# Ameek94/BOBE

Measured on AMD Instinct MI355X. Metric: GP fit+acquisition cycles/sec at N=4096 d=8, 65536 cands; Cholesky GF/s, higher is better.
Workload: dtype f64

## Files before the change

### bobe_amd/csrc/chol_kernels.hpp

```cpp
#pragma once
#include "kernels_common.hpp"

namespace bobe {

constexpr int PLD = 130;
constexpr int POTF2_DLD = 17;

template <bool LOWER = false, int NWAVES = 4>
__device__ __forceinline__ void block_load(double* S, const double* __restrict__ G, int64_t ld) {
  const int lane = threadIdx.x & 63, wave = threadIdx.x >> 6;
  constexpr int NI = TILE / NWAVES;
  v2d v[NI];
#pragma unroll
  for (int i = 0; i < NI; ++i) {
    const int r = NWAVES * i + wave;
    const int c = LOWER ? ((2 * lane <= r) ? 2 * lane : (r & ~1)) : 2 * lane;
    v[i] = *reinterpret_cast<const v2d*>(G + (int64_t)r * ld + c);
  }
#pragma unroll
  for (int i = 0; i < NI; ++i) *reinterpret_cast<v2d*>(S + (NWAVES * i + wave) * PLD + 2 * lane) = v[i];
}
__device__ __forceinline__ void block_store_lower(const double* S, double* __restrict__ G, int64_t ld) {
  const int lane = threadIdx.x & 63, wave = threadIdx.x >> 6;
#pragma unroll 8
// ... 598 lines not shown
}

__global__ __launch_bounds__(256) void k_copy_diag(double* __restrict__ A, int64_t lda, int64_t bsA,
                                                   const double* __restrict__ diag, int64_t bsD, int first) {
  const int blk = first + blockIdx.x;
  const double* src = diag + blockIdx.y * bsD + (int64_t)blk * TILE * TILE;
  double* dst = A + blockIdx.y * bsA + ((int64_t)blk * TILE) * lda + (int64_t)blk * TILE;
  const int lane = threadIdx.x & 63, wave = threadIdx.x >> 6;
#pragma unroll 8
  for (int i = 0; i < 32; ++i) {
    const int r = 4 * i + wave;
    *reinterpret_cast<v2d*>(dst + (int64_t)r * lda + 2 * lane) = *reinterpret_cast<const v2d*>(src + r * TILE + 2 * lane);
  }
}

template <int T, int BK>
__global__ __launch_bounds__(256) void k_syrk_trail(double* __restrict__ A, int64_t lda, int k0, int k1, int first,
                                                    int colmode, int n, int64_t bsA = 0, int per = 0,
                                                    const int* __restrict__ colk0 = nullptr, int far_col = 0, int ncol = 0) {
  extern __shared__ double smem[];
  A += blockIdx.y * bsA;
  int a, b;
  if (colmode == 0) {
    if (per > 0) {
      const int t = xcd_share(blockIdx.x, per);
      if (t >= n * (n + 1) / 2) return;
      tri_grouped(t, n, a, b);
    } else {
      tri_decode(blockIdx.x, a, b);
    }
  } else {
    const int S = colmode == 1 ? TILE / T : ncol;
// ... 2 lines not shown
    for (int c = 0; c < S - 1; ++c)
      if (b == c && idx >= n - c) {
        idx -= n - c;
        b = c + 1;
      }
    a = b + idx;
  }
  if (colk0) {
    const int col = first + (b * T) / TILE;
    if (col >= far_col) k0 = colk0[col];
    if (k0 >= k1) return;
  }
  const int64_t base = (int64_t)first * TILE;
  v4d acc[T / 32][T / 32];
  load_tile<T, T>(acc, A, lda, base + (int64_t)a * T, base + (int64_t)b * T);
  gemm_tile<KC, KC, T, T, BK, true>(acc, A, lda, base + (int64_t)a * T, A, lda, base + (int64_t)b * T,
                                    (int64_t)k0 * TILE, (int64_t)k1 * TILE, smem);
  store_tile<T, T>(acc, A, lda, base + (int64_t)a * T, base + (int64_t)b * T, 1.0, 0.0);
}


template <int T>
__device__ __forceinline__ bool tri_find(const TriProb* __restrict__ probs, int nprob, int bid, TriProb& p, int& e0,
                                         int& e1) {
  constexpr int S = (TILE / T) * (TILE / T);
  for (int q = 0; q < nprob; ++q) {
    const TriProb c = probs[q];
    const int nt = (c.hi - c.mid) * (c.mid - c.lo) * S;
    const int nw = (T == 128) ? nt : nt / 2;
    const int o = (T == 128) ? c.off : c.off * S / 2;
    if (bid >= o && bid < o + nw) {
      p = c;
      e0 = bid - o;
      e1 = (T == 128) ? -1 : nt - 1 - e0;
      return true;
    }
  }
  return false;
}

template <int T>
__global__ __launch_bounds__(256, 2) void k_trtri_T(const double* __restrict__ L, int64_t ldl,
                                                    const double* __restrict__ Linv, int64_t ldi,
                                                    double* __restrict__ Tmp, int64_t ldt,
                                                    const TriProb* __restrict__ probs, int nprob, int64_t bsA = 0,
                                                    int64_t bsL = 0, int64_t bsT = 0, int per = 0) {
  extern __shared__ double smem[];
  L += blockIdx.y * bsA;
  Linv += blockIdx.y * bsL;
  Tmp += blockIdx.y * bsT;
  TriProb p;
  int e[2];
  if (!tri_find<T>(probs, nprob, xcd_share(blockIdx.x, per), p, e[0], e[1])) return;
  const int rows = (p.hi - p.mid) * (TILE / T), w = (p.mid - p.lo) * (TILE / T);
  for (int u = 0; u < 2; ++u) {
    if (e[u] < 0) continue;
    int ti, tj;
    if (per > 0) {
      rect_grouped(e[u], w, rows, tj, ti);
    } else {
      tj = e[u] / rows, ti = e[u] % rows;
    }
    const int64_t m0 = (int64_t)p.mid * TILE + (int64_t)ti * T, n0 = (int64_t)p.lo * TILE + (int64_t)tj * T;
    v4d acc[T / 32][T / 32];
    acc_zero(acc);
    gemm_tile<KC, RC, T, T, TileCfg<T>::bk>(acc, L, ldl, m0, Linv, ldi, n0, n0, (int64_t)p.mid * TILE, smem);
    store_tile<T, T>(acc, Tmp, ldt, m0, n0, 1.0, 0.0);
  }
}

template <int T>
__global__ __launch_bounds__(256, 2) void k_trtri_R(double* __restrict__ Linv, int64_t ldi,
                                                    const double* __restrict__ Tmp, int64_t ldt,
                                                    const TriProb* __restrict__ probs, int nprob, int64_t bsL = 0,
                                                    int64_t bsT = 0, int per = 0) {
  extern __shared__ double smem[];
  Linv += blockIdx.y * bsL;
  Tmp += blockIdx.y * bsT;
  TriProb p;
  int e[2];
  if (!tri_find<T>(probs, nprob, xcd_share(blockIdx.x, per), p, e[0], e[1])) return;
  const int rows = (p.hi - p.mid) * (TILE / T), w = (p.mid - p.lo) * (TILE / T);
  for (int u = 0; u < 2; ++u) {
    if (e[u] < 0) continue;
    int ti, tj;
    if (per > 0) {
      rect_grouped(e[u], rows, w, ti, tj);
      ti = rows - 1 - ti;
    } else {
      ti = rows - 1 - e[u] / w, tj = e[u] % w;
    }
    const int64_t m0 = (int64_t)p.mid * TILE + (int64_t)ti * T, n0 = (int64_t)p.lo * TILE + (int64_t)tj * T;
    v4d acc[T / 32][T / 32];
    acc_zero(acc);
    gemm_tile<KC, RC, T, T, TileCfg<T>::bk>(acc, Linv, ldi, m0, Tmp, ldt, n0, (int64_t)p.mid * TILE, m0 + T, smem);
    store_tile<T, T>(acc, Linv, ldi, m0, n0, -1.0, 0.0);
  }
}

__global__ __launch_bounds__(256, 2) void k_lauum_tiles32(const double* __restrict__ Linv, int64_t ldi, int64_t np,
                                                          double* __restrict__ Kinv, int64_t ldk, int64_t bsL, int64_t bsK,
                                                          int nbatch) {
  extern __shared__ double smem[];
  const int tile = (int)(blockIdx.x / nbatch), slot = (int)(blockIdx.x % nbatch);
  Linv += slot * bsL;
  Kinv += slot * bsK;
  int ti, tj;
  tri_decode(tile >> 2, ti, tj);
  const int r32 = 2 * ti + ((tile >> 1) & 1), c32 = 2 * tj + (tile & 1);
  v4d acc[1][1];
  acc_zero(acc);
  gemm_tile<RC, RC, 32, 32, BK32>(acc, Linv, ldi, (int64_t)r32 * 32, Linv, ldi, (int64_t)c32 * 32,
                                  (int64_t)(r32 > c32 ? r32 : c32) * 32, np, smem);
  store_tile<32, 32>(acc, Kinv, ldk, (int64_t)r32 * 32, (int64_t)c32 * 32, 1.0, 0.0);
}

template <int KERN, int DCAP, int T>
__global__ __launch_bounds__(256, 2) void k_lauum_grad(const double* __restrict__ Linv, int64_t ldi, int64_t np,
                                                       int64_t n, const double* __restrict__ alpha,
                                                       const double* __restrict__ XsT, int64_t ldx, Hyper h,
                                                       double* __restrict__ partial, double* __restrict__ Kinv,
                                                       int64_t ldk, const Hyper* __restrict__ hp = nullptr,
                                                       int64_t bsL = 0, int64_t bsV = 0, int64_t bsX = 0,
                                                       int64_t bsP = 0, int nbatch = 1, int from_kinv = 0, int64_t bsK = 0) {
  extern __shared__ double smem[];
  const int tile = (int)(blockIdx.x / nbatch), slot = (int)(blockIdx.x % nbatch);
  if (hp) h = hp[slot];
  Linv += slot * bsL;
  alpha += slot * bsV;
  XsT += slot * bsX;
  partial += slot * bsP;
  int ti, tj;
  tri_decode(tile, ti, tj);
  v4d acc[T / 32][T / 32];
  if (from_kinv) {
    load_tile<T, T>(acc, Kinv + slot * bsK, ldk, (int64_t)ti * T, (int64_t)tj * T);
  } else {
    acc_zero(acc);
    gemm_tile<RC, RC, T, T, TileCfg<T>::bk>(acc, Linv, ldi, (int64_t)ti * T, Linv, ldi, (int64_t)tj * T, (int64_t)ti * T, np,
                                            smem);
    if (Kinv) store_tile<T, T>(acc, Kinv, ldk, (int64_t)ti * T, (int64_t)tj * T, 1.0, 0.0);
  }
  double* xa = smem;
  double* xb = smem + MAX_D * T;
  double* aa = smem + 2 * MAX_D * T;
  double* ab = aa + T;
  double* red = ab + T;
  const int t = threadIdx.x;
  for (int e = t; e < h.d * T; e += 256) {
    const int j = e / T, c = e % T;
    xa[j * T + c] = XsT[j * ldx + (int64_t)ti * T + c];
    xb[j * T + c] = XsT[j * ldx + (int64_t)tj * T + c];
  }
  if (t < T) {
    aa[t] = alpha[(int64_t)ti * T + t];
// ... 51 lines not shown
```

### bobe_amd/csrc/gemm_f64.hpp

```cpp
#pragma once
#include <hip/hip_runtime.h>
#include <stdint.h>
#include <type_traits>

namespace bobe {

typedef double v4d __attribute__((ext_vector_type(4)));
typedef double v2d __attribute__((ext_vector_type(2)));

constexpr int TILE = 128;
constexpr int TK = 16;
constexpr int GEMM_THREADS = 256;

enum Layout { KC = 0, RC = 1 };

template <int L, int R, int BK>
struct Img {
  static constexpr int stride = (L == KC) ? (BK + 2) : (R + 16);
  static constexpr int doubles = (L == KC) ? R * (BK + 2) : BK * (R + 16);
};
constexpr int imax(int a, int b) { return a > b ? a : b; }
template <int TM, int TN, int BK>
constexpr int gemm_smem_doubles() {
  return 2 * (imax(Img<KC, TM, BK>::doubles, Img<RC, TM, BK>::doubles) +
// ... 307 lines not shown
    BOBE_STAMP_STEP();
    buf ^= 1;
    frags(fa[0], fb[0], smem + buf * (IA + IB), 0);
    __builtin_amdgcn_sched_barrier(0);
    mfmas(BK / 4 - 1);
    __builtin_amdgcn_sched_barrier(0);
    BOBE_STAMP(0);
  };
  const int64_t kd = TRIL ? (kend - TM > kbeg ? kend - TM : kbeg) : kend;
  for (int64_t k0 = kbeg; k0 < kd; k0 += BK) kstep(k0, std::false_type(), 0);
  if (TRIL)
    for (int64_t k0 = kd; k0 < kend; k0 += BK) kstep(k0, std::true_type(), (int)(k0 - (kend - TM)));
  BOBE_STAMPS_END(tid);
}

template <int TM = 128>
__device__ __forceinline__ int acc_row(int i, int r, int tid = threadIdx.x) {
  const int t = tid;
  return ((t >> 6) >> 1) * (TM / 2) + 16 * i + ((t & 63) >> 4) + 4 * r;
}
template <int TN = 128>
__device__ __forceinline__ int acc_col(int j, int tid = threadIdx.x) {
  const int t = tid;
  return ((t >> 6) & 1) * (TN / 2) + 16 * j + (t & 15);
}

template <int TM = 128, int TN = 128>
__device__ __forceinline__ void store_tile(const v4d (&acc)[TM / 32][TN / 32], double* __restrict__ C, int64_t ldc,
                                           int64_t m0, int64_t n0, double alpha, double beta, int tid = threadIdx.x) {
#pragma unroll
// ... 63 lines not shown
```

### bobe_amd/csrc/gp_factor.hip

```cpp
#include "gp_handle.hpp"

#include <chrono>

#include "chol_kernels.hpp"

using namespace bobe;

namespace bobe {

constexpr int SYRK32_BK = 128, SYRK64_BK = 16;
constexpr int SYRK32_SMEM = gemm_smem_doubles_exact<KC, KC, 32, 32, SYRK32_BK>() * 8 / 2;
constexpr int SYRK64_SMEM = gemm_smem_doubles_exact<KC, KC, 64, 64, SYRK64_BK>() * 8;

void configure_factor_kernels() {
  static bool done[64] = {false};
  int dev = 0;
  HIPCHK(hipGetDevice(&dev));
  if (dev < 0 || dev >= 64 || done[dev]) return;
  allow_big_lds(k_potf2<true>, POTF2_SMEM_BYTES);
  allow_big_lds(k_potf2<false>, POTF2_SMEM_BYTES);
  allow_big_lds(k_trti_diag, POTF2_SMEM_BYTES);
  allow_big_lds(k_trsm_panel, TRSM_SMEM_BYTES);
  allow_big_lds((k_chol_panel<false, 3>), POTF2_SMEM_BYTES);
  allow_big_lds((k_chol_panel<false, 4>), POTF2_SMEM_BYTES);
  allow_big_lds((k_chol_panel<true, 3>), POTF2_SMEM_BYTES);
  allow_big_lds((k_chol_panel<true, 4>), POTF2_SMEM_BYTES);
  allow_big_lds(k_trtri_T<128>, GEMM_SMEM_BYTES);
  allow_big_lds(k_trtri_R<128>, GEMM_SMEM_BYTES);
  allow_big_lds(k_syrk_trail<64, SYRK64_BK>, SYRK64_SMEM);
  allow_big_lds(k_syrk_trail<32, SYRK32_BK>, SYRK32_SMEM);
  allow_big_lds(k_trtri_T<64>, GEMM64_SMEM_BYTES);
  allow_big_lds(k_trtri_R<64>, GEMM64_SMEM_BYTES);
  allow_big_lds(k_trtri_T<32>, GEMM32_SMEM_BYTES);
  allow_big_lds(k_trtri_R<32>, GEMM32_SMEM_BYTES);
  allow_big_lds(k_lauum_tiles32, GEMM32_SMEM_BYTES);
  allow_big_lds(k_lauum_grad<0, 8, 64>, GEMM64_SMEM_BYTES);
  allow_big_lds(k_lauum_grad<0, 16, 64>, GEMM64_SMEM_BYTES);
  allow_big_lds(k_lauum_grad<0, 32, 64>, GEMM64_SMEM_BYTES);
  allow_big_lds(k_lauum_grad<1, 8, 64>, GEMM64_SMEM_BYTES);
  allow_big_lds(k_lauum_grad<1, 16, 64>, GEMM64_SMEM_BYTES);
  allow_big_lds(k_lauum_grad<1, 32, 64>, GEMM64_SMEM_BYTES);
  allow_big_lds(k_lauum_grad<0, 8, 128>, GEMM_SMEM_BYTES);
  allow_big_lds(k_lauum_grad<0, 16, 128>, GEMM_SMEM_BYTES);
  allow_big_lds(k_lauum_grad<0, 32, 128>, GEMM_SMEM_BYTES);
  allow_big_lds(k_lauum_grad<1, 8, 128>, GEMM_SMEM_BYTES);
  allow_big_lds(k_lauum_grad<1, 16, 128>, GEMM_SMEM_BYTES);
  allow_big_lds(k_lauum_grad<1, 32, 128>, GEMM_SMEM_BYTES);
  done[dev] = true;
}

const Tuning& tuning() {
  static Tuning t = [] {
    Tuning v{512, 600, 300, 1, BOBE_MAX_MLL_SLOTS, 2048, 1, 1, false, false, true, true};
    auto geti = [](const char* name, int& dst) {
      const char* e = std::getenv(name);
      if (e) dst = std::atoi(e);
      return e != nullptr;
    };
    geti("BOBE_SYRK32_BELOW", v.syrk32_below);
    geti("BOBE_TRTRI64", v.trtri64_below);
    geti("BOBE_PAIR_MIN", v.pair_min);
    geti("BOBE_LOCKSTEP_MIN_N", v.lockstep_min_n);
    v.mll_slots_set = geti("BOBE_MLL_SLOTS", v.mll_slots);
    geti("BOBE_GRAPH_MAX_N", v.graph_max_n);
    geti("BOBE_XCD_SHARES", v.xcd_shares);
    geti("BOBE_FILL", v.fill);
    v.trace = std::getenv("BOBE_TRACE") != nullptr;
    int reuse = 1;
    geti("BOBE_FACTOR_REUSE", reuse);
    v.factor_reuse = reuse != 0;
    int glds = 1;
    geti("BOBE_GEMM_GLDS", glds);
    v.gemm_glds = glds != 0;
    return v;
  }();
  return t;
}

double default_refine_kappa() {
  static const double v = [] {
    const char* e = std::getenv("BOBE_REFINE_KAPPA");
    return e ? std::atof(e) : 1e6;
  }();
  return v;
}

int default_solve_block() {
  static const int v = [] {
// ... 151 lines not shown
                   int ncols) {
  const Tuning& tu = tuning();
  const int rem = nb - first;
  if (rem <= 0 || (!colk0 && k1 <= k0)) return;
  const int kb = k1 - k0;
  const int n64 = 2 * rem, n32 = 4 * rem;
  const int nc64 = 2 * ncols;
  const int t64 = colmode == 2 ? nc64 * n64 - nc64 * (nc64 - 1) / 2 : (colmode ? 2 * n64 - 1 : n64 * (n64 + 1) / 2);
  const int t32 = colmode ? 4 * n32 - 6 : n32 * (n32 + 1) / 2;
  if (kb == 1 && !colk0 && colmode != 2 && B * t64 < tu.syrk32_below) {
    hipLaunchKernelGGL((k_syrk_trail<32, SYRK32_BK>), dim3(t32, B), dim3(256), SYRK32_SMEM, stream, a, Np, k0, k1, first,
                       colmode, n32, bsA, 0, (const int*)nullptr, 0, 0);
    return;
  }
  const TileGrid tg = colmode ? TileGrid{t64, 0} : tile_grid(t64);
  hipLaunchKernelGGL((k_syrk_trail<64, SYRK64_BK>), dim3(tg.grid, B), dim3(256), SYRK64_SMEM, stream, a, Np, k0, k1, first,
                     colmode, n64, bsA, tg.per, colk0, far_col, nc64);
}

int bobe_gp::panel_strips(int B, int rr) const {
  return B * panel_workgroups(rr, 3) <= std::max(num_cus, 1) ? 3 : 4;
}

bool bobe_gp::fill_pays(int B) const {
  const int f = tuning().fill;
  if (f == 0 || in_slot) return false;
  if (f == 2) return true;
  return nb >= 28 && 20 * B * panel_workgroups(nb - 1, panel_strips(B, nb - 1)) <= 7 * std::max(num_cus, 1);
}

const bobe_gp::CholPlan& bobe_gp::chol_plan(int B, bool fill) {
  const Tuning& tu = tuning();
// ... 191 lines not shown
  aside_first = 1 << 30;
  aside_dg = nullptr;
  prof_end(BOBE_PROF_TRTRI);
  for (int dd = (int)depths.size() - 1; dd >= 0; --dd) {
    const Depth& D = depths[dd];
    const TriProb* pr = static_cast<const TriProb*>(probs.p) + D.first;
    prof_begin(BOBE_PROF_TRTRI);
    if (B * 2 * D.nblocks <= std::max(num_cus, 1)) {
      const TileGrid tg = tile_grid(8 * D.nblocks);
      hipLaunchKernelGGL(k_trtri_T<32>, dim3(tg.grid, B), dim3(256), GEMM32_SMEM_BYTES, stream, a, Np,
                         (const double*)linv, Np, tmp, Np, pr, D.count, bsA, bsL, bsT, tg.per);
      hipLaunchKernelGGL(k_trtri_R<32>, dim3(tg.grid, B), dim3(256), GEMM32_SMEM_BYTES, stream, linv, Np,
                         (const double*)tmp, Np, pr, D.count, bsL, bsT, tg.per);
    } else if (D.nblocks < tu.trtri64_below) {
      const TileGrid tg = tile_grid(2 * D.nblocks);
      hipLaunchKernelGGL(k_trtri_T<64>, dim3(tg.grid, B), dim3(256), GEMM64_SMEM_BYTES, stream, a, Np,
                         (const double*)linv, Np, tmp, Np, pr, D.count, bsA, bsL, bsT, tg.per);
      hipLaunchKernelGGL(k_trtri_R<64>, dim3(tg.grid, B), dim3(256), GEMM64_SMEM_BYTES, stream, linv, Np,
                         (const double*)tmp, Np, pr, D.count, bsL, bsT, tg.per);
    } else {
      hipLaunchKernelGGL(k_trtri_T<128>, dim3(D.nblocks, B), dim3(256), GEMM_SMEM_BYTES, stream, a, Np,
                         (const double*)linv, Np, tmp, Np, pr, D.count, bsA, bsL, bsT);
      hipLaunchKernelGGL(k_trtri_R<128>, dim3(D.nblocks, B), dim3(256), GEMM_SMEM_BYTES, stream, linv, Np,
                         (const double*)tmp, Np, pr, D.count, bsL, bsT);
    }
    prof_end(BOBE_PROF_TRTRI);
  }
  LAUNCH_CHECK();
}

int bobe_gp::lauum(const Hyper& h, const double* linv, const double* al, const double* xst, double* kinv_out, int dcap,
                   const Hyper* hdev, double* gp_out, int B, int64_t bsL, int64_t bsV, int64_t bsX, int64_t bsP,
                   double* scratch, int64_t bsS) {
  const bool small = nb * (nb + 1) / 2 < LAUUM64_BELOW;
  const int nt = small ? 2 * nb : nb;
  const int ntiles = nt * (nt + 1) / 2;
  double* gpo = gp_out ? gp_out : gpart.d();
  const bool split = small && scratch && !kinv_out && B * ntiles < 4 * std::max(num_cus, 1);
  double* kio = split ? scratch : kinv_out;
  const int64_t bsK = split ? bsS : 0;
  prof_begin(BOBE_PROF_LAUUM);
  if (split) {
    hipLaunchKernelGGL(k_lauum_tiles32, dim3(4 * ntiles * B), dim3(256), GEMM32_SMEM_BYTES, stream, linv, Np, Np, scratch, Np,
                       bsL, bsS, B);
  }
#define LG(KE, DC, TT)                                                                                          \
  hipLaunchKernelGGL((k_lauum_grad<KE, DC, TT>), dim3(ntiles * B), dim3(256),                                   \
                     (TT == 128 ? GEMM_SMEM_BYTES : GEMM64_SMEM_BYTES), stream, linv, Np, Np, N, al, xst, Np, h, \
                     gpo, kio, Np, hdev, bsL, bsV, bsX, bsP, B, split ? 1 : 0, bsK)
#define LGD(KE, TT)                                                                 \
  do {                                                                              \
    if (dcap == 8) LG(KE, 8, TT); else if (dcap == 16) LG(KE, 16, TT); else LG(KE, 32, TT); \
  } while (0)
  if (h.kern == 0) {
    if (small) LGD(0, 64); else LGD(0, 128);
  } else {
    if (small) LGD(1, 64); else LGD(1, 128);
  }
  prof_end(BOBE_PROF_LAUUM);
#undef LGD
#undef LG
  LAUNCH_CHECK();
  return ntiles;
}
// ... 729 lines not shown
```

### bobe_amd/csrc/gp_handle.hpp

```cpp
#pragma once
#include "../../include/bobe_gp.h"

#include <hip/hip_runtime.h>

#include <algorithm>
#include <array>
#include <climits>
#include <cmath>
#include <cstdio>
#include <cstdlib>
#include <cstring>
#include <map>
#include <mutex>
#include <stdexcept>
#include <string>
#include <vector>

#include "gemm_f64.hpp"
#include "gp_types.hpp"

namespace bobe {

struct Err : std::runtime_error {
  int code;
// ... 50 lines not shown
}
inline bool pivots_resolved(double min_diag, double floor) { return min_diag * min_diag >= floor; }
double default_pivot_floor_ulp();
double default_refine_kappa();
int default_solve_block();
int default_solve_panel();
int64_t default_solve_chunk();

template <typename K>
void allow_big_lds(K kernel, int bytes) {
  HIPCHK(hipFuncSetAttribute(reinterpret_cast<const void*>(kernel), hipFuncAttributeMaxDynamicSharedMemorySize, bytes));
}

struct Tuning {
  int syrk32_below, trtri64_below, pair_min, lockstep_min_n, mll_slots, graph_max_n, xcd_shares, fill;
  bool mll_slots_set, trace, factor_reuse, gemm_glds;
};
const Tuning& tuning();

constexpr int LAUUM64_BELOW = 1200;
constexpr int FILL_NEAR = 2;
constexpr int FILL_CHUNK = 3;
constexpr int FILL_SLACK = 16;
constexpr int FILL_PHASE = 1024;

struct TileGrid { int grid, per; };
inline TileGrid tile_grid(int ntiles) {
  if (!tuning().xcd_shares || ntiles < 256) return {ntiles, 0};
  const int per = (ntiles + 7) / 8;
  return {8 * per, per};
}
// ... 288 lines not shown
```

### bobe_amd/csrc/gp_sweep.hip

```cpp
#include "gp_handle.hpp"

#include "sweep_kernels.hpp"

using namespace bobe;

namespace bobe {
void configure_sweep_kernels() {
  static bool done[64] = {false};
  int dev = 0;
  HIPCHK(hipGetDevice(&dev));
  if (dev < 0 || dev >= 64 || done[dev]) return;
  allow_big_lds(k_trimul<true>, GEMM_SMEM_BYTES);
  allow_big_lds(k_trimul<false>, GEMM_SMEM_BYTES);
  allow_big_lds(k_trimul_t, GEMM_SMEM_BYTES);
  allow_big_lds(k_trimul_v64, GEMM64_SMEM_BYTES);
  allow_big_lds(k_trimul_t64, GEMM64_SMEM_BYTES);
  allow_big_lds(k_blk_step, GEMM_SMEM_BYTES);
  allow_big_lds(k_cross_vv<128, true>, GEMM_SMEM_BYTES);
  allow_big_lds(k_cross_vv<128, false>, GEMM_SMEM_BYTES);
  allow_big_lds(k_cross_vv<64>, GEMM64_SMEM_BYTES);
  done[dev] = true;
}

static auto trimul_kernel() { return tuning().gemm_glds ? k_trimul<true> : k_trimul<false>; }
static auto cross_vv128_kernel() { return tuning().gemm_glds ? k_cross_vv<128, true> : k_cross_vv<128, false>; }
}

void bobe_gp::decide_refinement(double min_diag) {
  const double piv = min_diag * min_diag;
  refine_v = refine_kappa >= 0.0 && piv > 0.0 && (hyp.kvar + hyp.noise) / piv > refine_kappa;
}

void bobe_gp::solve_v(double* B, int64_t ldb, int64_t ncp, double* V, int64_t ldv, double* qp, int64_t ldq) {
  if (!refine_v) {
    hipLaunchKernelGGL(trimul_kernel(), dim3((unsigned)(ncp / TILE), (unsigned)nb), dim3(256), GEMM_SMEM_BYTES, stream,
                       (const double*)Linv.d(), Np, nb, (const double*)B, ldb, V, ldv, qp, ldq, (const double*)nullptr,
                       (int64_t)0, 0, (double*)nullptr, (int64_t)0, (const double*)nullptr, (int64_t)0, 0, 1 << 30);
    return;
  }
  if (!V) throw Err(BOBE_ERR_STATE, "solve_v: the blocked substitution needs a buffer for V");
// ... 9 lines not shown
    const int p1 = std::min(nb, p0 + pt);
    if (p0 > 0) step(p0, p1 - p0, 0, p0, 0, 0);
    for (int t0 = p0; t0 < p1; t0 += bt) {
      const int t1 = std::min(p1, t0 + bt);
      step(0, 0, 0, 0, t0, t1 - t0);
      if (t1 < p1) step(t1, p1 - t1, t0, t1, 0, 0);
    }
  }
}

void bobe_gp::prepare_z(const double* Z, int64_t M, int64_t Mp, bool need_w) {
  const bool host_z = !is_device_ptr(Z);
  const bool few = (Mp / TILE) * nb < 2 * std::max(num_cus, 1);
  auto make_w = [&]() {
    if (few)
      hipLaunchKernelGGL(k_trimul_t64, dim3((unsigned)(Mp / 64), (unsigned)(2 * nb)), dim3(256), GEMM64_SMEM_BYTES, stream,
                         (const double*)Linv.d(), Np, 2 * nb, (const double*)VZ.d(), Mp, WZ.d(), Mp);
    else
      hipLaunchKernelGGL(k_trimul_t, dim3((unsigned)(Mp / TILE), (unsigned)nb), dim3(256), GEMM_SMEM_BYTES, stream,
                         (const double*)Linv.d(), Np, nb, (const double*)VZ.d(), Mp, WZ.d(), Mp);
    LAUNCH_CHECK();
    wz_ready = true;
  };
  if (host_z && z_seen_m == M && std::memcmp(z_seen.data(), Z, (size_t)M * d * sizeof(double)) == 0) {
    if (need_w && !wz_ready) make_w();
    return;
  }
  forget_z();
  if (host_z) z_seen.assign(Z, Z + (size_t)M * d);
  const double* zin = fetch(Z, (size_t)M * d, z_stage);
  ZsT.ensure((size_t)d * Mp * sizeof(double));
  kXZ.ensure((size_t)Np * Mp * sizeof(double));
  VZ.ensure((size_t)Np * Mp * sizeof(double));
  WZ.ensure((size_t)Np * Mp * sizeof(double));
  basez.ensure((size_t)Mp * sizeof(double));
  qpart.ensure((size_t)2 * nb * (Mp > chunk ? Mp : chunk) * sizeof(double));
  scale(zin, M, Mp, hyp, ZsT.d(), Mp);
  kernel_matrix_cross(XsT.d(), Np, N, Np, ZsT.d(), Mp, M, Mp, hyp, kXZ.d(), Mp);
  if (refine_v) {
    solve_v(kXZ.d(), Mp, Mp, VZ.d(), Mp, qpart.d(), Mp);
    hipLaunchKernelGGL(k_predict_finalize, dim3((unsigned)((Mp + 255) / 256)), dim3(256), 0, stream,
                       (const double*)qpart.d(), Mp, nb, Mp, hyp.kvar + hyp.noise, 0, basez.d(), (double*)nullptr);
  } else if (few) {
    const int nt = 2 * nb;
    hipLaunchKernelGGL(k_trimul_v64, dim3((unsigned)(Mp / 64), (unsigned)nt), dim3(256), GEMM64_SMEM_BYTES, stream,
                       (const double*)Linv.d(), Np, nt, (const double*)kXZ.d(), Mp, VZ.d(), Mp, qpart.d(), Mp);
    hipLaunchKernelGGL(k_predict_finalize, dim3((unsigned)((Mp + 255) / 256)), dim3(256), 0, stream,
                       (const double*)qpart.d(), Mp, nt, Mp, hyp.kvar + hyp.noise, 0, basez.d(), (double*)nullptr);
  } else {
    hipLaunchKernelGGL(trimul_kernel(), dim3((unsigned)(Mp / TILE), (unsigned)nb), dim3(256), GEMM_SMEM_BYTES, stream,
                       (const double*)Linv.d(), Np, nb, (const double*)kXZ.d(), Mp, VZ.d(), Mp, qpart.d(), Mp,
                       (const double*)nullptr, (int64_t)0, 0, (double*)nullptr, (int64_t)0, (const double*)nullptr,
                       (int64_t)0, 0, 1 << 30);
    hipLaunchKernelGGL(k_predict_finalize, dim3((unsigned)((Mp + 255) / 256)), dim3(256), 0, stream,
                       (const double*)qpart.d(), Mp, nb, Mp, hyp.kvar + hyp.noise, 0, basez.d(), (double*)nullptr);
  }
  LAUNCH_CHECK();
  if (need_w) make_w();
  if (host_z) z_seen_m = M;
}
// ... 25 lines not shown
  qpart.ensure((size_t)nb * (Mp > CH ? Mp : CH) * sizeof(double));
  part.ensure((size_t)nb * (Np > CH ? Np : CH) * sizeof(double));
  if (do_wip) pv.ensure((size_t)Mp * SC * sizeof(double));
  if ((do_wip || refine_v) && !cand_is_z) vxc.ensure((size_t)Np * CH * sizeof(double));
  const bool fuse_cross = do_wip && !refine_v && C > CH;
  if (fuse_cross) vxc2.ensure((size_t)Np * CH * sizeof(double));
  double* vbuf[2] = {vxc.d(), fuse_cross ? vxc2.d() : vxc.d()};
  int vsel = 0;
  struct { bool valid; const double* V; int64_t ncp; double* cross; } pend = {false, nullptr, 0, nullptr};
  auto cross_alone = [&](const double* Vc, int64_t ncp_, double* cross_out, int64_t ldvc) {
    prof_begin(BOBE_PROF_CROSSVV);
    if ((int64_t)nzt * (ncp_ / TILE) >= 2 * std::max(num_cus, 1))
      hipLaunchKernelGGL(cross_vv128_kernel(), dim3((unsigned)(ncp_ / TILE), (unsigned)nzt), dim3(256), GEMM_SMEM_BYTES, stream,
                         (const double*)VZ.d(), Mp, Vc, ldvc, Np, cross_out, SC);
    else
      hipLaunchKernelGGL(k_cross_vv<64>, dim3((unsigned)(ncp_ / 64), (unsigned)(Mp / 64)), dim3(256), GEMM64_SMEM_BYTES,
                         stream, (const double*)VZ.d(), Mp, Vc, ldvc, Np, cross_out, SC);
    prof_end(BOBE_PROF_CROSSVV);
  };
  double* d_mean = out_dev(mean, C, o_mean);
  double* d_var = out_dev(var, C, o_var);
  double* d_wipv = nullptr;
  double* d_wipstd = nullptr;
  if (do_wip) {
    if (need_v) {
      if (wipv) d_wipv = out_dev(wipv, C, o_wipv);
      else { o_wipv.ensure(C * sizeof(double)); d_wipv = o_wipv.d(); }
    }
    if (need_s) {
      if (wipstd) d_wipstd = out_dev(wipstd, C, o_wipstd);
      else { o_wipstd.ensure(C * sizeof(double)); d_wipstd = o_wipstd.d(); }
// ... 471 lines not shown
```

### bobe_amd/csrc/sweep_kernels.hpp

```cpp
#pragma once
#include "kernels_common.hpp"

namespace bobe {

template <bool GLDS>
__global__ __launch_bounds__(256, 2) void k_trimul(const double* __restrict__ Linv, int64_t ldi, int nb,
                                                   const double* __restrict__ B, int64_t ldb, double* __restrict__ V,
                                                   int64_t ldv, double* __restrict__ qpart, int64_t ldq,
                                                   const double* __restrict__ VZ, int64_t ldw, int nzt,
                                                   double* __restrict__ crossT, int64_t ldx,
                                                   const double* __restrict__ Bx = nullptr, int64_t ldbx = 0, int ncx = 0,
                                                   int ncv = 1 << 30) {
  extern __shared__ double smem[];
  const int tc = blockIdx.x;
  v4d acc[4][4];
  acc_zero(acc);
  if ((int)blockIdx.y < nzt) {
    if (tc >= ncx) return;
    const int tz = blockIdx.y;
    if constexpr (GLDS)
      gemm_tile128_glds<RC, RC>(acc, VZ, ldw, (int64_t)tz * TILE, Bx, ldbx, (int64_t)tc * TILE, 0, (int64_t)nb * TILE, smem);
    else
      gemm_tile<RC, RC>(acc, VZ, ldw, (int64_t)tz * TILE, Bx, ldbx, (int64_t)tc * TILE, 0, (int64_t)nb * TILE, smem);
    store_tile(acc, crossT, ldx, (int64_t)tz * TILE, (int64_t)tc * TILE, 1.0, 0.0);
// ... 102 lines not shown
template <int T, bool GLDS = false>
__global__ __launch_bounds__(256, 2) void k_cross_vv(const double* __restrict__ VZ, int64_t ldz,
                                                     const double* __restrict__ V, int64_t ldv, int64_t kend,
                                                     double* __restrict__ crossT, int64_t ldx) {
  extern __shared__ double smem[];
  const int tc = blockIdx.x, tz = blockIdx.y;
  v4d acc[T / 32][T / 32];
  acc_zero(acc);
  if constexpr (T == 128) {
    if constexpr (GLDS)
      gemm_tile128_glds<RC, RC>(acc, VZ, ldz, (int64_t)tz * TILE, V, ldv, (int64_t)tc * TILE, 0, kend, smem);
    else
      gemm_tile<RC, RC>(acc, VZ, ldz, (int64_t)tz * TILE, V, ldv, (int64_t)tc * TILE, 0, kend, smem);
    store_tile(acc, crossT, ldx, (int64_t)tz * TILE, (int64_t)tc * TILE, 1.0, 0.0);
  } else {
    gemm_tile<RC, RC, 64, 64, BK64>(acc, VZ, ldz, (int64_t)tz * 64, V, ldv, (int64_t)tc * 64, 0, kend, smem);
    store_tile<64, 64>(acc, crossT, ldx, (int64_t)tz * 64, (int64_t)tc * 64, 1.0, 0.0);
  }
}

__global__ __launch_bounds__(256, 2) void k_trimul_t(const double* __restrict__ Linv, int64_t ldi, int nb,
                                                  const double* __restrict__ V, int64_t ldv, double* __restrict__ W,
                                                  int64_t ldw) {
  extern __shared__ double smem[];
  const int ti = blockIdx.y;
  const int tc = blockIdx.x;
  v4d acc[4][4];
  acc_zero(acc);
  gemm_tile<RC, RC>(acc, Linv, ldi, (int64_t)ti * TILE, V, ldv, (int64_t)tc * TILE, (int64_t)ti * TILE,
                    (int64_t)nb * TILE, smem);
  store_tile(acc, W, ldw, (int64_t)ti * TILE, (int64_t)tc * TILE, 1.0, 0.0);
}

__global__ __launch_bounds__(256, 2) void k_trimul_v64(const double* __restrict__ Linv, int64_t ldi, int nt,
                                                       const double* __restrict__ B, int64_t ldb, double* __restrict__ V,
                                                       int64_t ldv, double* __restrict__ qpart, int64_t ldq) {
  extern __shared__ double smem[];
  const int tc = blockIdx.x;
  const int ti = nt - 1 - (int)blockIdx.y;
  v4d acc[2][2];
  acc_zero(acc);
  gemm_tile<KC, RC, 64, 64, BK64>(acc, Linv, ldi, (int64_t)ti * 64, B, ldb, (int64_t)tc * 64, 0, (int64_t)(ti + 1) * 64, smem);
  store_tile<64, 64>(acc, V, ldv, (int64_t)ti * 64, (int64_t)tc * 64, 1.0, 0.0);
  const int t = threadIdx.x, lane = t & 63, wave = t >> 6;
  double* red = smem;
#pragma unroll
  for (int j = 0; j < 2; ++j) {
    double s = 0.0;
#pragma unroll
    for (int i = 0; i < 2; ++i)
#pragma unroll
      for (int r = 0; r < 4; ++r) s += acc[i][j][r] * acc[i][j][r];
    s += __shfl_xor(s, 16, 64);
    s += __shfl_xor(s, 32, 64);
    if (lane < 16) red[(wave >> 1) * 64 + (wave & 1) * 32 + 16 * j + lane] = s;
  }
  __syncthreads();
  if (t < 64) qpart[(int64_t)ti * ldq + (int64_t)tc * 64 + t] = red[t] + red[64 + t];
}

__global__ __launch_bounds__(256, 2) void k_trimul_t64(const double* __restrict__ Linv, int64_t ldi, int nt,
                                                       const double* __restrict__ V, int64_t ldv, double* __restrict__ W,
                                                       int64_t ldw) {
  extern __shared__ double smem[];
  const int ti = blockIdx.y;
  const int tc = blockIdx.x;
  v4d acc[2][2];
  acc_zero(acc);
  gemm_tile<RC, RC, 64, 64, BK64>(acc, Linv, ldi, (int64_t)ti * 64, V, ldv, (int64_t)tc * 64, (int64_t)ti * 64,
                                  (int64_t)nt * 64, smem);
  store_tile<64, 64>(acc, W, ldw, (int64_t)ti * 64, (int64_t)tc * 64, 1.0, 0.0);
}

template <int KERN, int DCAP>
__global__ __launch_bounds__(256) void k_wip_score(const double* __restrict__ crossT, int64_t ldx,
                                                   const double* __restrict__ CsT, int64_t ldc,
                                                   const double* __restrict__ ZsT, int64_t ldz, int64_t m,
                                                   const double* __restrict__ sc, const double* __restrict__ basez,
                                                   int64_t ncols, Hyper h, double ystd2, double* __restrict__ wipv,
                                                   double* __restrict__ wipstd, double* __restrict__ var_out,
                                                   int64_t ldvo) {
  extern __shared__ double zsm[];
  constexpr int ZT = 128;
  __shared__ double red[2][4][64];
  const int t = threadIdx.x, cx = t & 63, sl = t >> 6;
// ... 624 lines not shown
```

Baseline: 19.02.

## Add direct global-to-LDS buffer-load path for 64-tile f64 GEMMs

Adds a 64x64 f64 GEMM tile loop that stages A/B K-slices straight from global memory into LDS via buffer_load_lds with swizzled layouts, double-buffered, and wires it into syrk trail, trtri, lauum_grad, trimul and cross_vv 64-tile kernels behind a default-on tuning flag. It aims to remove the register round-trip and extra LDS writes of the existing staging path and to overlap loads with MFMA. It also raises syrk_trail occupancy hint to 2 blocks when enabled. It adds risk from the new swizzle indexing correctness and barrier placement.

```diff
diff --git a/bobe_amd/csrc/chol_kernels.hpp b/bobe_amd/csrc/chol_kernels.hpp
--- a/bobe_amd/csrc/chol_kernels.hpp
+++ b/bobe_amd/csrc/chol_kernels.hpp
@@ -636,8 +636,8 @@
   }
 }
 
-template <int T, int BK>
-__global__ __launch_bounds__(256) void k_syrk_trail(double* __restrict__ A, int64_t lda, int k0, int k1, int first,
+template <int T, int BK, bool GLDS = false>
+__global__ __launch_bounds__(256, GLDS ? 2 : 1) void k_syrk_trail(double* __restrict__ A, int64_t lda, int k0, int k1, int first,
                                                     int colmode, int n, int64_t bsA = 0, int per = 0,
                                                     const int* __restrict__ colk0 = nullptr, int far_col = 0, int ncol = 0) {
   extern __shared__ double smem[];
@@ -670,8 +670,12 @@
   const int64_t base = (int64_t)first * TILE;
   v4d acc[T / 32][T / 32];
   load_tile<T, T>(acc, A, lda, base + (int64_t)a * T, base + (int64_t)b * T);
-  gemm_tile<KC, KC, T, T, BK, true>(acc, A, lda, base + (int64_t)a * T, A, lda, base + (int64_t)b * T,
-                                    (int64_t)k0 * TILE, (int64_t)k1 * TILE, smem);
+  if constexpr (GLDS && T == 64 && BK == 16)
+    gemm_tile64_glds<KC, KC, true>(acc, A, lda, base + (int64_t)a * T, A, lda, base + (int64_t)b * T, (int64_t)k0 * TILE,
+                                   (int64_t)k1 * TILE, smem);
+  else
+    gemm_tile<KC, KC, T, T, BK, true>(acc, A, lda, base + (int64_t)a * T, A, lda, base + (int64_t)b * T,
+                                      (int64_t)k0 * TILE, (int64_t)k1 * TILE, smem);
   store_tile<T, T>(acc, A, lda, base + (int64_t)a * T, base + (int64_t)b * T, 1.0, 0.0);
 }
 
@@ -695,7 +699,7 @@
   return false;
 }
 
-template <int T>
+template <int T, bool GLDS = false>
 __global__ __launch_bounds__(256, 2) void k_trtri_T(const double* __restrict__ L, int64_t ldl,
                                                     const double* __restrict__ Linv, int64_t ldi,
                                                     double* __restrict__ Tmp, int64_t ldt,
@@ -720,12 +724,15 @@
     const int64_t m0 = (int64_t)p.mid * TILE + (int64_t)ti * T, n0 = (int64_t)p.lo * TILE + (int64_t)tj * T;
     v4d acc[T / 32][T / 32];
     acc_zero(acc);
-    gemm_tile<KC, RC, T, T, TileCfg<T>::bk>(acc, L, ldl, m0, Linv, ldi, n0, n0, (int64_t)p.mid * TILE, smem);
+    if constexpr (GLDS && T == 64)
+      gemm_tile64_glds<KC, RC>(acc, L, ldl, m0, Linv, ldi, n0, n0, (int64_t)p.mid * TILE, smem);
+    else
+      gemm_tile<KC, RC, T, T, TileCfg<T>::bk>(acc, L, ldl, m0, Linv, ldi, n0, n0, (int64_t)p.mid * TILE, smem);
     store_tile<T, T>(acc, Tmp, ldt, m0, n0, 1.0, 0.0);
   }
 }
 
-template <int T>
+template <int T, bool GLDS = false>
 __global__ __launch_bounds__(256, 2) void k_trtri_R(double* __restrict__ Linv, int64_t ldi,
                                                     const double* __restrict__ Tmp, int64_t ldt,
                                                     const TriProb* __restrict__ probs, int nprob, int64_t bsL = 0,
@@ -749,7 +756,10 @@
     const int64_t m0 = (int64_t)p.mid * TILE + (int64_t)ti * T, n0 = (int64_t)p.lo * TILE + (int64_t)tj * T;
     v4d acc[T / 32][T / 32];
     acc_zero(acc);
-    gemm_tile<KC, RC, T, T, TileCfg<T>::bk>(acc, Linv, ldi, m0, Tmp, ldt, n0, (int64_t)p.mid * TILE, m0 + T, smem);
+    if constexpr (GLDS && T == 64)
+      gemm_tile64_glds<KC, RC>(acc, Linv, ldi, m0, Tmp, ldt, n0, (int64_t)p.mid * TILE, m0 + T, smem);
+    else
+      gemm_tile<KC, RC, T, T, TileCfg<T>::bk>(acc, Linv, ldi, m0, Tmp, ldt, n0, (int64_t)p.mid * TILE, m0 + T, smem);
     store_tile<T, T>(acc, Linv, ldi, m0, n0, -1.0, 0.0);
   }
 }
@@ -771,7 +781,7 @@
   store_tile<32, 32>(acc, Kinv, ldk, (int64_t)r32 * 32, (int64_t)c32 * 32, 1.0, 0.0);
 }
 
-template <int KERN, int DCAP, int T>
+template <int KERN, int DCAP, int T, bool GLDS = false>
 __global__ __launch_bounds__(256, 2) void k_lauum_grad(const double* __restrict__ Linv, int64_t ldi, int64_t np,
                                                        int64_t n, const double* __restrict__ alpha,
                                                        const double* __restrict__ XsT, int64_t ldx, Hyper h,
@@ -793,8 +803,11 @@
     load_tile<T, T>(acc, Kinv + slot * bsK, ldk, (int64_t)ti * T, (int64_t)tj * T);
   } else {
     acc_zero(acc);
-    gemm_tile<RC, RC, T, T, TileCfg<T>::bk>(acc, Linv, ldi, (int64_t)ti * T, Linv, ldi, (int64_t)tj * T, (int64_t)ti * T, np,
-                                            smem);
+    if constexpr (GLDS && T == 64)
+      gemm_tile64_glds<RC, RC>(acc, Linv, ldi, (int64_t)ti * T, Linv, ldi, (int64_t)tj * T, (int64_t)ti * T, np, smem);
+    else
+      gemm_tile<RC, RC, T, T, TileCfg<T>::bk>(acc, Linv, ldi, (int64_t)ti * T, Linv, ldi, (int64_t)tj * T, (int64_t)ti * T,
+                                              np, smem);
     if (Kinv) store_tile<T, T>(acc, Kinv, ldk, (int64_t)ti * T, (int64_t)tj * T, 1.0, 0.0);
   }
   double* xa = smem;
diff --git a/bobe_amd/csrc/gemm_f64.hpp b/bobe_amd/csrc/gemm_f64.hpp
--- a/bobe_amd/csrc/gemm_f64.hpp
+++ b/bobe_amd/csrc/gemm_f64.hpp
@@ -345,6 +345,95 @@
   BOBE_STAMPS_END(tid);
 }
 
+constexpr int IMG64_DOUBLES = 64 * 16;
+constexpr int GEMM64_GLDS_SMEM_DOUBLES = 4 * IMG64_DOUBLES;
+static_assert(GEMM64_GLDS_SMEM_DOUBLES * 8 <= GEMM64_SMEM_BYTES, "the 64-tile LDS images must fit GEMM64_SMEM_BYTES");
+
+template <int L>
+__device__ __forceinline__ void glds_stage64(const double* __restrict__ p, int64_t ld, int64_t r0, int64_t k0, double* img,
+                                             int wave, int lane) {
+  const double* base = (L == KC) ? p + r0 * ld + k0 : p + k0 * ld + r0;
+  const __amdgpu_buffer_rsrc_t rs = __builtin_amdgcn_make_buffer_rsrc((void*)base, 0, 0x7fffffff, 0x00020000);
+#pragma unroll
+  for (int i = 0; i < 2; ++i) {
+    const int g = wave + 4 * i;
+    unsigned off;
+    if (L == KC) {
+      const int r = 8 * g + (lane >> 3);
+      off = (unsigned)((r * ld + 2 * ((lane & 7) ^ ((r >> 1) & 7))) * 8);
+    } else {
+      const int h = lane >> 5;
+      off = (unsigned)(((2 * g + h) * ld + 2 * ((lane & 31) ^ (8 * h))) * 8);
+    }
+    __builtin_amdgcn_raw_ptr_buffer_load_lds(rs, (__attribute__((address_space(3))) void*)(img + 128 * g), 16, off, 0, 0, 0);
+  }
+}
+
+template <int L>
+__device__ __forceinline__ double frag_read64(const double* img, int woff, int s, int ks, int lane) {
+  if (L == KC) {
+    const int h = (lane >> 5) ^ ((lane & 15) >> 1);
+    return img[(woff + 16 * s + (lane & 15)) * 16 + 2 * ((2 * ks) ^ h) + ((lane >> 4) & 1)];
+  } else {
+    return img[(4 * ks + (lane >> 4)) * 64 + ((woff + 16 * s + (lane & 15)) ^ (((lane >> 4) & 1) << 4))];
+  }
+}
+
+template <int LA, int LB, bool NEGA = false>
+__device__ __forceinline__ void gemm_tile64_glds(v4d (&acc)[2][2], const double* __restrict__ A, int64_t lda, int64_t m0,
+                                                 const double* __restrict__ B, int64_t ldb, int64_t n0, int64_t kbeg,
+                                                 int64_t kend, double* smem, int tid = threadIdx.x) {
+  constexpr int BK = 16;
+  static_assert(BK64 == BK, "gemm_tile64_glds is the BK = 16 loop");
+  constexpr int IA = IMG64_DOUBLES, IB = IMG64_DOUBLES;
+  const int lane = tid & 63;
+  const int wave = __builtin_amdgcn_readfirstlane(tid >> 6);
+  const int wm = (wave >> 1) * 32;
+  const int wn = (wave & 1) * 32;
+  if (kend <= kbeg) return;
+  auto stage = [&](int64_t k0, int b) {
+    double* ia = smem + b * (IA + IB);
+    glds_stage64<LA>(A, lda, m0, k0, ia, wave, lane);
+    glds_stage64<LB>(B, ldb, n0, k0, ia + IA, wave, lane);
+  };
+  double fa[2][2], fb[2][2];
+  auto frags = [&](double (&a)[2], double (&b)[2], const double* ia, int ks) {
+#pragma unroll
+    for (int s = 0; s < 2; ++s) a[s] = frag_read64<LA>(ia, wm, s, ks, lane);
+#pragma unroll
+    for (int s = 0; s < 2; ++s) b[s] = frag_read64<LB>(ia + IA, wn, s, ks, lane);
+  };
+  auto mfmas = [&](int ks) {
+#pragma unroll
+    for (int i = 0; i < 2; ++i) {
+      const double a = NEGA ? -fa[ks & 1][i] : fa[ks & 1][i];
+#pragma unroll
+      for (int j = 0; j < 2; ++j) acc[i][j] = __builtin_amdgcn_mfma_f64_16x16x4f64(a, fb[ks & 1][j], acc[i][j], 0, 0, 0);
+    }
+  };
+  stage(kbeg, 0);
+  __syncthreads();
+  frags(fa[0], fb[0], smem, 0);
+  int buf = 0;
+  for (int64_t k0 = kbeg; k0 < kend; k0 += BK) {
+    stage(k0 + BK < kend ? k0 + BK : k0, buf ^ 1);
+    const double* ia = smem + buf * (IA + IB);
+#pragma unroll
+    for (int ks = 0; ks < BK / 4 - 1; ++ks) {
+      frags(fa[(ks + 1) & 1], fb[(ks + 1) & 1], ia, ks + 1);
+      __builtin_amdgcn_sched_barrier(0);
+      mfmas(ks);
+      __builtin_amdgcn_sched_barrier(0);
+    }
+    __syncthreads();
+    buf ^= 1;
+    frags(fa[0], fb[0], smem + buf * (IA + IB), 0);
+    __builtin_amdgcn_sched_barrier(0);
+    mfmas(BK / 4 - 1);
+    __builtin_amdgcn_sched_barrier(0);
+  }
+}
+
 template <int TM = 128>
 __device__ __forceinline__ int acc_row(int i, int r, int tid = threadIdx.x) {
   const int t = tid;
diff --git a/bobe_amd/csrc/gp_factor.hip b/bobe_amd/csrc/gp_factor.hip
--- a/bobe_amd/csrc/gp_factor.hip
+++ b/bobe_amd/csrc/gp_factor.hip
@@ -28,9 +28,12 @@
   allow_big_lds(k_trtri_T<128>, GEMM_SMEM_BYTES);
   allow_big_lds(k_trtri_R<128>, GEMM_SMEM_BYTES);
   allow_big_lds(k_syrk_trail<64, SYRK64_BK>, SYRK64_SMEM);
+  allow_big_lds(k_syrk_trail<64, SYRK64_BK, true>, SYRK64_SMEM);
   allow_big_lds(k_syrk_trail<32, SYRK32_BK>, SYRK32_SMEM);
   allow_big_lds(k_trtri_T<64>, GEMM64_SMEM_BYTES);
   allow_big_lds(k_trtri_R<64>, GEMM64_SMEM_BYTES);
+  allow_big_lds(k_trtri_T<64, true>, GEMM64_SMEM_BYTES);
+  allow_big_lds(k_trtri_R<64, true>, GEMM64_SMEM_BYTES);
   allow_big_lds(k_trtri_T<32>, GEMM32_SMEM_BYTES);
   allow_big_lds(k_trtri_R<32>, GEMM32_SMEM_BYTES);
   allow_big_lds(k_lauum_tiles32, GEMM32_SMEM_BYTES);
@@ -40,6 +43,12 @@
   allow_big_lds(k_lauum_grad<1, 8, 64>, GEMM64_SMEM_BYTES);
   allow_big_lds(k_lauum_grad<1, 16, 64>, GEMM64_SMEM_BYTES);
   allow_big_lds(k_lauum_grad<1, 32, 64>, GEMM64_SMEM_BYTES);
+  allow_big_lds(k_lauum_grad<0, 8, 64, true>, GEMM64_SMEM_BYTES);
+  allow_big_lds(k_lauum_grad<0, 16, 64, true>, GEMM64_SMEM_BYTES);
+  allow_big_lds(k_lauum_grad<0, 32, 64, true>, GEMM64_SMEM_BYTES);
+  allow_big_lds(k_lauum_grad<1, 8, 64, true>, GEMM64_SMEM_BYTES);
+  allow_big_lds(k_lauum_grad<1, 16, 64, true>, GEMM64_SMEM_BYTES);
+  allow_big_lds(k_lauum_grad<1, 32, 64, true>, GEMM64_SMEM_BYTES);
   allow_big_lds(k_lauum_grad<0, 8, 128>, GEMM_SMEM_BYTES);
   allow_big_lds(k_lauum_grad<0, 16, 128>, GEMM_SMEM_BYTES);
   allow_big_lds(k_lauum_grad<0, 32, 128>, GEMM_SMEM_BYTES);
@@ -51,7 +60,7 @@
 
 const Tuning& tuning() {
   static Tuning t = [] {
-    Tuning v{512, 600, 300, 1, BOBE_MAX_MLL_SLOTS, 2048, 1, 1, false, false, true, true};
+    Tuning v{512, 600, 300, 1, BOBE_MAX_MLL_SLOTS, 2048, 1, 1, false, false, true, true, true};
     auto geti = [](const char* name, int& dst) {
       const char* e = std::getenv(name);
       if (e) dst = std::atoi(e);
@@ -72,6 +81,9 @@
     int glds = 1;
     geti("BOBE_GEMM_GLDS", glds);
     v.gemm_glds = glds != 0;
+    int glds64 = 1;
+    geti("BOBE_GEMM64_GLDS", glds64);
+    v.gemm64_glds = glds64 != 0;
     return v;
   }();
   return t;
@@ -253,8 +265,9 @@
     return;
   }
   const TileGrid tg = colmode ? TileGrid{t64, 0} : tile_grid(t64);
-  hipLaunchKernelGGL((k_syrk_trail<64, SYRK64_BK>), dim3(tg.grid, B), dim3(256), SYRK64_SMEM, stream, a, Np, k0, k1, first,
-                     colmode, n64, bsA, tg.per, colk0, far_col, nc64);
+  const auto k64 = tu.gemm64_glds ? k_syrk_trail<64, SYRK64_BK, true> : k_syrk_trail<64, SYRK64_BK, false>;
+  hipLaunchKernelGGL(k64, dim3(tg.grid, B), dim3(256), SYRK64_SMEM, stream, a, Np, k0, k1, first, colmode, n64, bsA, tg.per,
+                     colk0, far_col, nc64);
 }
 
 int bobe_gp::panel_strips(int B, int rr) const {
@@ -476,9 +489,11 @@
                          (const double*)tmp, Np, pr, D.count, bsL, bsT, tg.per);
     } else if (D.nblocks < tu.trtri64_below) {
       const TileGrid tg = tile_grid(2 * D.nblocks);
-      hipLaunchKernelGGL(k_trtri_T<64>, dim3(tg.grid, B), dim3(256), GEMM64_SMEM_BYTES, stream, a, Np,
+      const auto kT = tu.gemm64_glds ? k_trtri_T<64, true> : k_trtri_T<64, false>;
+      const auto kR = tu.gemm64_glds ? k_trtri_R<64, true> : k_trtri_R<64, false>;
+      hipLaunchKernelGGL(kT, dim3(tg.grid, B), dim3(256), GEMM64_SMEM_BYTES, stream, a, Np,
                          (const double*)linv, Np, tmp, Np, pr, D.count, bsA, bsL, bsT, tg.per);
-      hipLaunchKernelGGL(k_trtri_R<64>, dim3(tg.grid, B), dim3(256), GEMM64_SMEM_BYTES, stream, linv, Np,
+      hipLaunchKernelGGL(kR, dim3(tg.grid, B), dim3(256), GEMM64_SMEM_BYTES, stream, linv, Np,
                          (const double*)tmp, Np, pr, D.count, bsL, bsT, tg.per);
     } else {
       hipLaunchKernelGGL(k_trtri_T<128>, dim3(D.nblocks, B), dim3(256), GEMM_SMEM_BYTES, stream, a, Np,
@@ -506,10 +521,11 @@
     hipLaunchKernelGGL(k_lauum_tiles32, dim3(4 * ntiles * B), dim3(256), GEMM32_SMEM_BYTES, stream, linv, Np, Np, scratch, Np,
                        bsL, bsS, B);
   }
+  const bool g64 = tuning().gemm64_glds;
 #define LG(KE, DC, TT)                                                                                          \
-  hipLaunchKernelGGL((k_lauum_grad<KE, DC, TT>), dim3(ntiles * B), dim3(256),                                   \
-                     (TT == 128 ? GEMM_SMEM_BYTES : GEMM64_SMEM_BYTES), stream, linv, Np, Np, N, al, xst, Np, h, \
-                     gpo, kio, Np, hdev, bsL, bsV, bsX, bsP, B, split ? 1 : 0, bsK)
+  hipLaunchKernelGGL((g64 ? k_lauum_grad<KE, DC, TT, TT == 64> : k_lauum_grad<KE, DC, TT, false>), dim3(ntiles * B), \
+                     dim3(256), (TT == 128 ? GEMM_SMEM_BYTES : GEMM64_SMEM_BYTES), stream, linv, Np, Np, N, al, xst,   \
+                     Np, h, gpo, kio, Np, hdev, bsL, bsV, bsX, bsP, B, split ? 1 : 0, bsK)
 #define LGD(KE, TT)                                                                 \
   do {                                                                              \
     if (dcap == 8) LG(KE, 8, TT); else if (dcap == 16) LG(KE, 16, TT); else LG(KE, 32, TT); \
diff --git a/bobe_amd/csrc/gp_handle.hpp b/bobe_amd/csrc/gp_handle.hpp
--- a/bobe_amd/csrc/gp_handle.hpp
+++ b/bobe_amd/csrc/gp_handle.hpp
@@ -88,7 +88,7 @@
 
 struct Tuning {
   int syrk32_below, trtri64_below, pair_min, lockstep_min_n, mll_slots, graph_max_n, xcd_shares, fill;
-  bool mll_slots_set, trace, factor_reuse, gemm_glds;
+  bool mll_slots_set, trace, factor_reuse, gemm_glds, gemm64_glds;
 };
 const Tuning& tuning();
 
diff --git a/bobe_amd/csrc/gp_sweep.hip b/bobe_amd/csrc/gp_sweep.hip
--- a/bobe_amd/csrc/gp_sweep.hip
+++ b/bobe_amd/csrc/gp_sweep.hip
@@ -13,17 +13,23 @@
   allow_big_lds(k_trimul<true>, GEMM_SMEM_BYTES);
   allow_big_lds(k_trimul<false>, GEMM_SMEM_BYTES);
   allow_big_lds(k_trimul_t, GEMM_SMEM_BYTES);
-  allow_big_lds(k_trimul_v64, GEMM64_SMEM_BYTES);
-  allow_big_lds(k_trimul_t64, GEMM64_SMEM_BYTES);
+  allow_big_lds(k_trimul_v64<true>, GEMM64_SMEM_BYTES);
+  allow_big_lds(k_trimul_v64<false>, GEMM64_SMEM_BYTES);
+  allow_big_lds(k_trimul_t64<true>, GEMM64_SMEM_BYTES);
+  allow_big_lds(k_trimul_t64<false>, GEMM64_SMEM_BYTES);
   allow_big_lds(k_blk_step, GEMM_SMEM_BYTES);
   allow_big_lds(k_cross_vv<128, true>, GEMM_SMEM_BYTES);
   allow_big_lds(k_cross_vv<128, false>, GEMM_SMEM_BYTES);
-  allow_big_lds(k_cross_vv<64>, GEMM64_SMEM_BYTES);
+  allow_big_lds(k_cross_vv<64, true>, GEMM64_SMEM_BYTES);
+  allow_big_lds(k_cross_vv<64, false>, GEMM64_SMEM_BYTES);
   done[dev] = true;
 }
 
 static auto trimul_kernel() { return tuning().gemm_glds ? k_trimul<true> : k_trimul<false>; }
 static auto cross_vv128_kernel() { return tuning().gemm_glds ? k_cross_vv<128, true> : k_cross_vv<128, false>; }
+static auto cross_vv64_kernel() { return tuning().gemm64_glds ? k_cross_vv<64, true> : k_cross_vv<64, false>; }
+static auto trimul_v64_kernel() { return tuning().gemm64_glds ? k_trimul_v64<true> : k_trimul_v64<false>; }
+static auto trimul_t64_kernel() { return tuning().gemm64_glds ? k_trimul_t64<true> : k_trimul_t64<false>; }
 }
 
 void bobe_gp::decide_refinement(double min_diag) {
@@ -63,7 +69,7 @@
   const bool few = (Mp / TILE) * nb < 2 * std::max(num_cus, 1);
   auto make_w = [&]() {
     if (few)
-      hipLaunchKernelGGL(k_trimul_t64, dim3((unsigned)(Mp / 64), (unsigned)(2 * nb)), dim3(256), GEMM64_SMEM_BYTES, stream,
+      hipLaunchKernelGGL(trimul_t64_kernel(), dim3((unsigned)(Mp / 64), (unsigned)(2 * nb)), dim3(256), GEMM64_SMEM_BYTES, stream,
                          (const double*)Linv.d(), Np, 2 * nb, (const double*)VZ.d(), Mp, WZ.d(), Mp);
     else
       hipLaunchKernelGGL(k_trimul_t, dim3((unsigned)(Mp / TILE), (unsigned)nb), dim3(256), GEMM_SMEM_BYTES, stream,
@@ -92,7 +98,7 @@
                        (const double*)qpart.d(), Mp, nb, Mp, hyp.kvar + hyp.noise, 0, basez.d(), (double*)nullptr);
   } else if (few) {
     const int nt = 2 * nb;
-    hipLaunchKernelGGL(k_trimul_v64, dim3((unsigned)(Mp / 64), (unsigned)nt), dim3(256), GEMM64_SMEM_BYTES, stream,
+    hipLaunchKernelGGL(trimul_v64_kernel(), dim3((unsigned)(Mp / 64), (unsigned)nt), dim3(256), GEMM64_SMEM_BYTES, stream,
                        (const double*)Linv.d(), Np, nt, (const double*)kXZ.d(), Mp, VZ.d(), Mp, qpart.d(), Mp);
     hipLaunchKernelGGL(k_predict_finalize, dim3((unsigned)((Mp + 255) / 256)), dim3(256), 0, stream,
                        (const double*)qpart.d(), Mp, nt, Mp, hyp.kvar + hyp.noise, 0, basez.d(), (double*)nullptr);
@@ -148,7 +154,7 @@
       hipLaunchKernelGGL(cross_vv128_kernel(), dim3((unsigned)(ncp_ / TILE), (unsigned)nzt), dim3(256), GEMM_SMEM_BYTES, stream,
                          (const double*)VZ.d(), Mp, Vc, ldvc, Np, cross_out, SC);
     else
-      hipLaunchKernelGGL(k_cross_vv<64>, dim3((unsigned)(ncp_ / 64), (unsigned)(Mp / 64)), dim3(256), GEMM64_SMEM_BYTES,
+      hipLaunchKernelGGL(cross_vv64_kernel(), dim3((unsigned)(ncp_ / 64), (unsigned)(Mp / 64)), dim3(256), GEMM64_SMEM_BYTES,
                          stream, (const double*)VZ.d(), Mp, Vc, ldvc, Np, cross_out, SC);
     prof_end(BOBE_PROF_CROSSVV);
   };
diff --git a/bobe_amd/csrc/sweep_kernels.hpp b/bobe_amd/csrc/sweep_kernels.hpp
--- a/bobe_amd/csrc/sweep_kernels.hpp
+++ b/bobe_amd/csrc/sweep_kernels.hpp
@@ -140,7 +140,10 @@
       gemm_tile<RC, RC>(acc, VZ, ldz, (int64_t)tz * TILE, V, ldv, (int64_t)tc * TILE, 0, kend, smem);
     store_tile(acc, crossT, ldx, (int64_t)tz * TILE, (int64_t)tc * TILE, 1.0, 0.0);
   } else {
-    gemm_tile<RC, RC, 64, 64, BK64>(acc, VZ, ldz, (int64_t)tz * 64, V, ldv, (int64_t)tc * 64, 0, kend, smem);
+    if constexpr (GLDS)
+      gemm_tile64_glds<RC, RC>(acc, VZ, ldz, (int64_t)tz * 64, V, ldv, (int64_t)tc * 64, 0, kend, smem);
+    else
+      gemm_tile<RC, RC, 64, 64, BK64>(acc, VZ, ldz, (int64_t)tz * 64, V, ldv, (int64_t)tc * 64, 0, kend, smem);
     store_tile<64, 64>(acc, crossT, ldx, (int64_t)tz * 64, (int64_t)tc * 64, 1.0, 0.0);
   }
 }
@@ -158,6 +161,7 @@
   store_tile(acc, W, ldw, (int64_t)ti * TILE, (int64_t)tc * TILE, 1.0, 0.0);
 }
 
+template <bool GLDS>
 __global__ __launch_bounds__(256, 2) void k_trimul_v64(const double* __restrict__ Linv, int64_t ldi, int nt,
                                                        const double* __restrict__ B, int64_t ldb, double* __restrict__ V,
                                                        int64_t ldv, double* __restrict__ qpart, int64_t ldq) {
@@ -166,7 +170,11 @@
   const int ti = nt - 1 - (int)blockIdx.y;
   v4d acc[2][2];
   acc_zero(acc);
-  gemm_tile<KC, RC, 64, 64, BK64>(acc, Linv, ldi, (int64_t)ti * 64, B, ldb, (int64_t)tc * 64, 0, (int64_t)(ti + 1) * 64, smem);
+  if constexpr (GLDS)
+    gemm_tile64_glds<KC, RC>(acc, Linv, ldi, (int64_t)ti * 64, B, ldb, (int64_t)tc * 64, 0, (int64_t)(ti + 1) * 64, smem);
+  else
+    gemm_tile<KC, RC, 64, 64, BK64>(acc, Linv, ldi, (int64_t)ti * 64, B, ldb, (int64_t)tc * 64, 0, (int64_t)(ti + 1) * 64,
+                                    smem);
   store_tile<64, 64>(acc, V, ldv, (int64_t)ti * 64, (int64_t)tc * 64, 1.0, 0.0);
   const int t = threadIdx.x, lane = t & 63, wave = t >> 6;
   double* red = smem;
@@ -185,6 +193,7 @@
   if (t < 64) qpart[(int64_t)ti * ldq + (int64_t)tc * 64 + t] = red[t] + red[64 + t];
 }
 
+template <bool GLDS>
 __global__ __launch_bounds__(256, 2) void k_trimul_t64(const double* __restrict__ Linv, int64_t ldi, int nt,
                                                        const double* __restrict__ V, int64_t ldv, double* __restrict__ W,
                                                        int64_t ldw) {
@@ -193,8 +202,12 @@
   const int tc = blockIdx.x;
   v4d acc[2][2];
   acc_zero(acc);
-  gemm_tile<RC, RC, 64, 64, BK64>(acc, Linv, ldi, (int64_t)ti * 64, V, ldv, (int64_t)tc * 64, (int64_t)ti * 64,
-                                  (int64_t)nt * 64, smem);
+  if constexpr (GLDS)
+    gemm_tile64_glds<RC, RC>(acc, Linv, ldi, (int64_t)ti * 64, V, ldv, (int64_t)tc * 64, (int64_t)ti * 64, (int64_t)nt * 64,
+                             smem);
+  else
+    gemm_tile<RC, RC, 64, 64, BK64>(acc, Linv, ldi, (int64_t)ti * 64, V, ldv, (int64_t)tc * 64, (int64_t)ti * 64,
+                                    (int64_t)nt * 64, smem);
   store_tile<64, 64>(acc, W, ldw, (int64_t)ti * 64, (int64_t)tc * 64, 1.0, 0.0);
 }
 
```

Result: faster. 19.73 (median of 6 runs) (+3.7%).
